# s-elkazdadi/ddp-pinocchio

Measured on AMD Instinct MI355X. Metric: DDP iterations/sec (fwd+bwd sweep), Talos nq=38 T=200, higher is better.
Workload: dtype f64

## Files before the change

### ddp_pinocchio_amd/csrc/lin_static.hip

```cpp
#include <float.h>
#include <math.h>
#include <stdlib.h>

#include <type_traits>
#include <utility>

#include "internal.h"
#include "lin_common.h"
#include "rbd.h"

#ifndef DEV_NO_EMIT
#define DEV_NO_EMIT 0
#endif
namespace {

struct TopoTalos38 {
  static constexpr int N = 38;
  static constexpr int parent[N] = {-1, 0, 1, 2, 3, 4,
                                    5, 6, 7, 8, 9, 10,
                                    5, 12, 13, 14, 15, 16,
                                    5, 18,
                                    19, 20, 21, 22, 23, 24, 25, 26,
                                    19, 28, 29, 30, 31, 32, 33, 34,
                                    19, 36};
  static constexpr int prismatic[N] = {1, 1, 1, 0, 0, 0, 0, 0, 0, 0, 0, 0, 0, 0, 0, 0, 0, 0, 0,
                                       0, 0, 0, 0, 0, 0, 0, 0, 0, 0, 0, 0, 0, 0, 0, 0, 0, 0, 0};
};

struct TopoChain6 {
  static constexpr int N = 6;
  static constexpr int parent[N] = {-1, 0, 1, 2, 3, 4};
  static constexpr int prismatic[N] = {0, 0, 0, 0, 0, 0};
};

}
#include "topo_extra.h"
namespace {

template <class T> constexpr bool has_child(int k) {
  for (int c = k + 1; c < T::N; ++c) if (T::parent[c] == k) return true;
  return false;
}
template <class T> constexpr int largest_child(int k) {
  int r = -1;
  for (int c = k + 1; c < T::N; ++c) if (T::parent[c] == k) r = c;
  return r;
}
template <class T> constexpr bool first_contrib(int k) { return T::parent[k] >= 0 && largest_child<T>(T::parent[k]) == k; }

template <class T>
bool topo_matches(const DevModel& m) {
  if (m.kind != DDP_HIP_MODEL_TREE || m.nv != T::N) return false;
  for (int i = 0; i < T::N; ++i)
    if (m.parent[i] != T::parent[i] || (m.jtype[i] == DDP_HIP_JOINT_PRISMATIC) != (T::prismatic[i] != 0)) return false;
  return true;
}

template <class T>
struct TauState {
  double acc[T::N][6];
  double uu[T::N];
};

template <class T, int K, int QS>
__device__ __forceinline__ void tau_up(const DevModel& m, const double* __restrict__ qc, const double* __restrict__ vc,
                                       double tauK, TauState<T>& s) {
  constexpr int o = T::prismatic[K] ? 3 : 0;
  const double* E = qc + K * QS;
  const double* r = E + 9;
  const double* U = E + 12;
  const double dinv = E[18];
  const double* pA0 = vc + K * rbd::VC_STRIDE + 6;
  const double* Iac = vc + K * rbd::VC_STRIDE + 12;
  const double* a = m.axis[K];
  double pAi[6];
  if constexpr (has_child<T>(K)) {
#pragma unroll
    for (int k = 0; k < 6; ++k) pAi[k] = s.acc[K][k];
  } else {
#pragma unroll
    for (int k = 0; k < 6; ++k) pAi[k] = pA0[k];
  }
  double sp = 0;
#pragma unroll
  for (int k = 0; k < 3; ++k) sp += a[k] * pAi[o + k];
  const double ui = tauK - sp;
  s.uu[K] = ui;
  constexpr int par = T::parent[K];
  if constexpr (par >= 0) {
    double pa[6], fp[6];
#pragma unroll
    for (int k = 0; k < 6; ++k) pa[k] = pAi[k] + Iac[k] + U[k] * (ui * dinv);
    rbd::xform_force_T(E, r, pa, fp);
    if constexpr (first_contrib<T>(K)) {
      const double* pp0 = vc + par * rbd::VC_STRIDE + 6;
#pragma unroll
      for (int k = 0; k < 6; ++k) s.acc[par][k] = pp0[k] + fp[k];
    } else {
#pragma unroll
      for (int k = 0; k < 6; ++k) s.acc[par][k] += fp[k];
    }
  }
  if constexpr (QS == rbd::QC_STRIDE || (K % 2) == 0) __builtin_amdgcn_sched_barrier(0);
}

template <class T, int K, int QS>
__device__ __forceinline__ void tau_down(const DevModel& m, const double* __restrict__ qc, const double* __restrict__ vc,
                                         TauState<T>& s) {
  constexpr int o = T::prismatic[K] ? 3 : 0;
  const double* E = qc + K * QS;
  const double* r = E + 9;
  const double* U = E + 12;
  const double dinv = E[18];
  const double* cb = vc + K * rbd::VC_STRIDE;
  double ap[6];
  constexpr int par = T::parent[K];
  if constexpr (par >= 0) rbd::xform_motion(E, r, s.acc[par], ap);
  else {
    const double a0[6] = {0, 0, 0, -m.gravity[0], -m.gravity[1], -m.gravity[2]};
    rbd::xform_motion(E, r, a0, ap);
  }
  double sum = 0;
#pragma unroll
  for (int k = 0; k < 6; ++k) { ap[k] += cb[k]; sum += U[k] * ap[k]; }
  const double qd = (s.uu[K] - sum) * dinv;
  s.uu[K] = qd;
  if constexpr (has_child<T>(K)) {
    const double* a = m.axis[K];
#pragma unroll
    for (int k = 0; k < 6; ++k) s.acc[K][k] = ap[k];
    s.acc[K][o] += a[0] * qd; s.acc[K][o + 1] += a[1] * qd; s.acc[K][o + 2] += a[2] * qd;
  }
  if constexpr (QS == rbd::QC_STRIDE || (K % 2) == 0) __builtin_amdgcn_sched_barrier(0);
}

template <class T, int QS, class TauFn, int... Ks>
__device__ __forceinline__ void tau_up_all(const DevModel& m, const double* __restrict__ qc, const double* __restrict__ vc, TauFn tau,
                                           TauState<T>& s, std::integer_sequence<int, Ks...>) {
  (tau_up<T, T::N - 1 - Ks, QS>(m, qc, vc, tau(T::N - 1 - Ks), s), ...);
}
template <class T, int QS, int HI, class TauFn, int... Ks>
__device__ __forceinline__ void tau_up_range(const DevModel& m, const double* __restrict__ qc, const double* __restrict__ vc, TauFn tau,
                                             TauState<T>& s, std::integer_sequence<int, Ks...>) {
  (tau_up<T, HI - Ks, QS>(m, qc, vc, tau(HI - Ks), s), ...);
}
template <class T, int QS, int... Ks>
__device__ __forceinline__ void tau_down_all(const DevModel& m, const double* __restrict__ qc, const double* __restrict__ vc,
                                             TauState<T>& s, std::integer_sequence<int, Ks...>) {
  (tau_down<T, Ks, QS>(m, qc, vc, s), ...);
}

constexpr int PS = 20;
template <int NV>
__device__ __forceinline__ void stage_placements(double* sp, const double* __restrict__ qc, int lane) {
  for (int idx = lane; idx < NV * 19; idx += LBS) {
    const int K = idx / 19, e = idx - K * 19;
    sp[K * PS + e] = qc[K * rbd::QC_STRIDE + e];
  }
}

template <int BYTES>
__device__ __forceinline__ unsigned int warm_block(const double* base, int lane) {
  typedef unsigned int u4 __attribute__((ext_vector_type(4)));
  const char* b = reinterpret_cast<const char*>(base);
  unsigned int sink = 0;
#pragma unroll
  for (int off = 0; off < BYTES; off += LBS * 16) {
    int o = off + lane * 16;
    o = o < BYTES - 16 ? o : BYTES - 16;
    const u4 v = *reinterpret_cast<const u4*>(b + o);
    sink ^= v.x ^ v.y ^ v.z ^ v.w;
  }
  return sink;
}

template <class T> constexpr bool parents_at_least(int from, int lo) {
  for (int k = from; k < T::N; ++k) if (T::parent[k] < lo) return false;
  return true;
}
template <class T> constexpr int stage_split() {
  for (int kh = T::N / 2; kh > 0; --kh) if (parents_at_least<T>(kh + 1, kh)) return kh;
  return 0;
}

template <int NV, int K0, int K1, bool WITH_V = true>
struct StageRegs {
  static constexpr int NPW = (K1 - K0) * 19, NVW = WITH_V ? (K1 - K0) * rbd::VC_STRIDE : 0;
  static constexpr int CP = (NPW + LBS - 1) / LBS, CV = (NVW + LBS - 1) / LBS;
  double rp[CP], rv[CV > 0 ? CV : 1];
  __device__ __forceinline__ void load(const double* __restrict__ qc, const double* __restrict__ vc, int lane) {
#pragma unroll
    for (int c = 0; c < CP; ++c) {
      int idx = c * LBS + lane;
      idx = idx < NPW ? idx : NPW - 1;
      const int K = K0 + idx / 19, e = idx % 19;
      rp[c] = qc[K * rbd::QC_STRIDE + e];
    }
#pragma unroll
    for (int c = 0; c < CV; ++c) {
      int idx = c * LBS + lane;
      idx = idx < NVW ? idx : NVW - 1;
      rv[c] = vc[K0 * rbd::VC_STRIDE + idx];
    }
  }
  __device__ __forceinline__ void park(double* sp, double* sv, int lane) const {
#pragma unroll
    for (int c = 0; c < CP; ++c) {
      int idx = c * LBS + lane;
      idx = idx < NPW ? idx : NPW - 1;
      const int K = K0 + idx / 19, e = idx % 19;
      sp[K * PS + e] = rp[c];
    }
#pragma unroll
    for (int c = 0; c < CV; ++c) {
      int idx = c * LBS + lane;
      idx = idx < NVW ? idx : NVW - 1;
      sv[K0 * rbd::VC_STRIDE + idx] = rv[c];
    }
  }
};

__device__ __forceinline__ void tri_index(int64_t q, int Wd, int& ii, int& jj) {
  int a = (int)floor(((2.0 * Wd - 1.0) - sqrt((2.0 * Wd - 1.0) * (2.0 * Wd - 1.0) - 8.0 * (double)q)) * 0.5);
  if (a < 0) a = 0;
  while ((int64_t)a * (2 * Wd - a - 1) / 2 > q) --a;
  while ((int64_t)(a + 1) * (2 * Wd - a - 2) / 2 <= q) ++a;
  ii = a;
  jj = (int)(q - (int64_t)a * (2 * Wd - a - 1) / 2) + a + 1;
}

template <int NV, int NP = LBS>
struct OutStage {
  double qdd[NP * (NV + 1)];
  int pij[NP];
};

template <int NV, int NP>
__device__ __forceinline__ void offdiag_emit(const LinParams& p, OutStage<NV, NP>& S, bool valid, int i, int j, int64_t bt,
                                             const double* __restrict__ xg, double dt, int pass = 0) {
  constexpr int n = 2 * NV, mm = NV;
  constexpr int RW = 16, NJ = (n + RW - 1) / RW, GRP = LBS / RW, PPG = NP / GRP, NB = NP == LBS ? 2 : 1;
  static_assert(PPG % NB == 0, "points per group");
  const double eps = sqrt(sqrt(DBL_EPSILON));
  const double eps2 = eps * eps;
  const int lane = threadIdx.x;
  if (lane / NP == pass) S.pij[lane % NP] = i | (j << 8) | ((valid ? 1 : 0) << 16);
  double* const fxx = p.fxx + bt * n * n * n;
  double* const fux = p.fux + bt * n * mm * n;
  double* const fuu = p.fuu + bt * n * mm * mm;
  const double* const fxb = p.fx + bt * n * n;
  const double* const fub = p.fu + bt * n * mm;
  __syncthreads();
  const int kk = lane % RW, grp = lane / RW;
  const double* f0 = p.f_val + bt * n;
  double f0k[NJ], xk[NJ], xvk[NJ];
#pragma unroll
  for (int jx = 0; jx < NJ; ++jx) {
    const int k = kk + RW * jx;
    const int kc = k < n ? k : n - 1;
    f0k[jx] = f0[kc];
    xk[jx] = xg[kc];
    xvk[jx] = kc < NV ? xg[NV + kc] : 0.0;
  }
  if (DEV_NO_EMIT) return;
  for (int pt = 0; pt < PPG; pt += NB) {
    double a1[NB][NJ], a2[NB][NJ], d1[NB][NJ], d2[NB][NJ];
    double* o0[NB];
    double* o1[NB];
    int ie[NB], je[NB], ee[NB];
#pragma unroll
    for (int u = 0; u < NB; ++u) {
      const int e = (pt + u) * GRP + grp;
      ee[u] = e;
      const int pk = S.pij[e];
      const int i1 = pk & 255, j1 = (pk >> 8) & 255;
      ie[u] = i1;
      je[u] = j1;
      const bool at_x_1 = i1 < n, at_x_2 = j1 < n;
      const int idx_1 = at_x_1 ? i1 : i1 - n, idx_2 = at_x_2 ? j1 : j1 - n;
      double* tensor;
      int L;
      if (at_x_1) { if (at_x_2) { tensor = fxx; L = n; } else { tensor = fux; L = mm; } }
      else { tensor = fuu; L = mm; }
      o0[u] = (pk >> 16) ? tensor + (int64_t)idx_2 * n + (int64_t)idx_1 * n * L : nullptr;
      o1[u] = ((pk >> 16) && at_x_1 == at_x_2 && !p.skip_qv_mirror) ? tensor + (int64_t)idx_1 * n + (int64_t)idx_2 * n * L : nullptr;
      if (o0[u]) {
        const double* q0 = at_x_1 ? fxb + (int64_t)idx_1 * n : fub + (int64_t)idx_1 * n;
        const double* q1 = at_x_2 ? fxb + (int64_t)idx_2 * n : fub + (int64_t)idx_2 * n;
        const double* q2 = at_x_1 ? fxx + (int64_t)idx_1 * n + (int64_t)idx_1 * n * n : fuu + (int64_t)idx_1 * n + (int64_t)idx_1 * n * mm;
        const double* q3 = at_x_2 ? fxx + (int64_t)idx_2 * n + (int64_t)idx_2 * n * n : fuu + (int64_t)idx_2 * n + (int64_t)idx_2 * n * mm;
#pragma unroll
        for (int jx = 0; jx < NJ; ++jx) {
          const int k = kk + RW * jx;
          const int kc = k < n ? k : n - 1;
          a1[u][jx] = q0[kc]; a2[u][jx] = q1[kc]; d1[u][jx] = q2[kc]; d2[u][jx] = q3[kc];
        }
      }
    }
#pragma unroll
    for (int u = 0; u < NB; ++u) {
      if (!o0[u]) continue;
#pragma unroll
      for (int jx = 0; jx < NJ; ++jx) {
        const int k = kk + RW * jx;
        if (k >= n) continue;
        if (p.skip_top && k < NV && !((ie[u] < n && ie[u] % NV == k) || (je[u] < n && je[u] % NV == k))) continue;
        double xs = k == ie[u] ? xk[jx] + eps : xk[jx];
        if (k == je[u]) xs = xs + eps;
        double fv;
        if (k < NV) {
          double xv = (NV + k) == ie[u] ? xvk[jx] + eps : xvk[jx];
          if (NV + k == je[u]) xv = xv + eps;
          const double vo = dt * xv;
          fv = xs + vo;
        } else {
          fv = xs + S.qdd[ee[u] * (NV + 1) + (k - NV)] * dt;
        }
        double df = fv - f0k[jx];
        df -= eps * a1[u][jx];
        df -= eps * a2[u][jx];
        df *= 2;
        const double val = 0.5 * (df / eps2 - d1[u][jx] - d2[u][jx]);
        o0[u][k] = val;
        if (o1[u]) o1[u][k] = val;
      }
    }
  }
}

template <int NV>
struct RowStage {
  double q[(NV + 2) * (NV + 1)];
};

template <int NV, bool DIAG_ROW, class ST>
__device__ __forceinline__ void rowblock_emit(const ST& S, int lane, int i, int jb, double* __restrict__ out, double* __restrict__ mirror,
                                              int64_t mstride, const double* __restrict__ a2, const double* __restrict__ d2, int64_t dstride,
                                              double dt, const double* __restrict__ f0g, const double* __restrict__ a1g,
                                              double* __restrict__ d1g, const double* __restrict__ xg, bool skip_top = false) {
  constexpr int n = 2 * NV, RW = 16, NJ = (n + RW - 1) / RW, CG = LBS / RW, NIT = (NV + CG - 1) / CG;
  const int r1 = i % NV;
  const double eps = sqrt(sqrt(DBL_EPSILON));
  const double eps2 = eps * eps;
  const int kk = lane % RW, cg = lane / RW;
  double xk[NJ], xvk[NJ], f0k[NJ], a1k[NJ], d1k[NJ];
#pragma unroll
  for (int j = 0; j < NJ; ++j) {
    const int k = kk + RW * j;
    const int kc = k < n ? k : n - 1;
    f0k[j] = f0g[kc];
    a1k[j] = a1g[kc];
    double x = xg[kc];
    if (kc == i) x = x + eps;
    xk[j] = x;
    double xv = xg[kc < NV ? NV + kc : kc];
    if (NV + kc == i) xv = xv + eps;
    xvk[j] = xv;
    if constexpr (DIAG_ROW) {
      double fv;
      if (kc < NV) {
        const double vo = dt * xv;
        fv = x + vo;
      } else {
        fv = x + S.q[NV * (NV + 1) + (kc - NV)] * dt;
      }
      double df = fv - f0k[j];
      df -= eps * a1k[j];
      df *= 2;
      const double dd = df / eps2;
      d1k[j] = dd;
      if (cg == 0 && k < n && !(skip_top && k < NV && k != r1)) d1g[k] = dd;
    } else {
      d1k[j] = d1g[kc];
    }
  }
  double va2[2][NJ], vd2[2][NJ];
  auto fetch = [&](int it, double (&A)[NJ], double (&D)[NJ]) {
    const int c = it * CG + cg;
    const int cc = c < NV ? c : NV - 1;
#pragma unroll
    for (int j = 0; j < NJ; ++j) {
      const int k = kk + RW * j;
      const int kc = k < n ? k : n - 1;
      A[j] = a2[kc + cc * n];
      D[j] = d2[kc + cc * dstride];
    }
  };
  auto form = [&](int it, const double (&A)[NJ], const double (&D)[NJ]) {
    const int c = it * CG + cg;
    const bool cv = c < NV;
    const int cc = cv ? c : NV - 1;
    const int jp = jb + cc;
#pragma unroll
    for (int j = 0; j < NJ; ++j) {
      const int k = kk + RW * j;
      if (!(cv && k < n)) continue;
      if (skip_top && k < NV && k != r1 && !(jp < n && jp % NV == k)) continue;
      double x = xk[j];
      if (k == jp) x = x + eps;
      double fv;
      if (k < NV) {
        double xv = xvk[j];
        if (NV + k == jp) xv = xv + eps;
        const double vo = dt * xv;
        fv = x + vo;
      } else {
        fv = x + S.q[cc * (NV + 1) + (k - NV)] * dt;
      }
      double df = fv - f0k[j];
      df -= eps * a1k[j];
      df -= eps * A[j];
      df *= 2;
      const double val = 0.5 * (df / eps2 - d1k[j] - D[j]);
      out[k + c * n] = val;
      if (mirror) mirror[k + c * mstride] = val;
    }
  };
  if (DEV_NO_EMIT) return;
  fetch(0, va2[0], vd2[0]);
  for (int it = 0; it < NIT; it += 2) {
    if (it + 1 < NIT) fetch(it + 1, va2[1], vd2[1]);
    form(it, va2[0], vd2[0]);
    if (it + 1 < NIT) {
      if (it + 2 < NIT) fetch(it + 2, va2[0], vd2[0]);
      form(it + 1, va2[1], vd2[1]);
    }
  }
}

template <class T, bool ROWS>
__global__ __launch_bounds__(LBS, ROWS ? 1 : 3) void lin_static_tau_kernel(LinParams p) {
  constexpr int nv = T::N, n = 2 * nv;
  constexpr int TRI = nv * (nv - 1) / 2, GU = (TRI + LBS - 1) / LBS, G = ROWS ? 2 * nv : GU;
  const int64_t bt = blockIdx.x / G;
  const int g = (int)(blockIdx.x % G) + (ROWS ? 0 : 2 * nv);
  const int lane = threadIdx.x;
  const int64_t Tn = p.d.T;
  const int b = (int)(bt / Tn);
  const int64_t t = bt % Tn;
  const DevModel& m = *p.model;
  int i, j, cfg, vcfg;
  bool valid;
  if (g < nv) { i = g; j = n + lane; cfg = 1 + g; vcfg = nv + 1 + g; valid = lane < nv; }
  else if (g < 2 * nv) { i = g; j = n + lane; cfg = 0; vcfg = 1 + (g - nv); valid = lane < nv; }
  else {
    const int pid = (g - 2 * nv) * LBS + lane;
    valid = pid < TRI;
    tri_index(valid ? pid : 0, nv, i, j);
    i += n; j += n; cfg = 0; vcfg = 0;
  }
  double eps = sqrt(sqrt(DBL_EPSILON));
  const double* __restrict__ qc = p.qcache + (bt * (nv + 1) + cfg) * (int64_t)nv * rbd::QC_STRIDE;
  const double* __restrict__ vc = p.vcache + (bt * (2 * nv + 1) + vcfg) * (int64_t)nv * rbd::VC_STRIDE;
  const double* __restrict__ xg = p.x + ((int64_t)b * (Tn + 1) + t) * n;
  const double* __restrict__ ug = p.u + ((int64_t)b * Tn + t) * nv;
  const int iu = i - n, ju = j - n;
  __shared__ union TauLds { double P[ROWS ? nv * PS + nv * rbd::VC_STRIDE : 1]; RowStage<nv> S; } s_lds;
  double* s_P = s_lds.P;
  unsigned int w = 0;
  double* s_V = s_P + nv * PS;
  constexpr int KH = ROWS ? stage_split<T>() : 0;
  StageRegs<nv, 0, (ROWS && KH > 0) ? KH : 1> lower;
  if constexpr (ROWS) {
    StageRegs<nv, KH, nv> upper;
    upper.load(qc, vc, lane);
    lower.load(qc, vc, lane);
    upper.park(s_P, s_V, lane);
    rbd::coop_sync<true>();
  } else {
    w = warm_block<nv * rbd::VC_STRIDE * 8>(vc, lane);
    w ^= warm_block<nv * rbd::QC_STRIDE * 8>(qc, lane);
  }
  if (w == 0x7fc01234u) eps = 0.0;
  TauState<T> s;
  auto tau = [&](int k) { double v = ug[k]; if (k == iu) v = v + eps; if (k == ju) v = v + eps; return v; };
  if constexpr (ROWS) {
    static_assert(!ROWS || parents_at_least<T>(KH + 1, KH), "the first half of the pass must not reach below record KH");
    tau_up_range<T, PS, nv - 1>(m, s_P, s_V, tau, s, std::make_integer_sequence<int, nv - 1 - KH>{});
    lower.park(s_P, s_V, lane);
    rbd::coop_sync<true>();
    tau_up_range<T, PS, KH>(m, s_P, s_V, tau, s, std::make_integer_sequence<int, KH + 1>{});
    tau_down_all<T, PS>(m, s_P, s_V, s, std::make_integer_sequence<int, nv>{});
  } else {
    tau_up_all<T, rbd::QC_STRIDE>(m, qc, vc, tau, s, std::make_integer_sequence<int, nv>{});
    tau_down_all<T, rbd::QC_STRIDE>(m, qc, vc, s, std::make_integer_sequence<int, nv>{});
  }
  __builtin_amdgcn_sched_barrier(0);
  typedef __attribute__((address_space(4))) const LinParams* kernarg_t;
  const kernarg_t kp = (kernarg_t)__builtin_amdgcn_kernarg_segment_ptr();
  if constexpr (ROWS) {
    RowStage<nv>& S = s_lds.S;
    const int mm = nv;
    __syncthreads();
    const int row = lane <= nv ? lane : nv + 1;
#pragma unroll
    for (int k = 0; k < nv; ++k) S.q[row * (nv + 1) + k] = s.uu[k];
    __syncthreads();
    rowblock_emit<nv, true>(S, lane, i, n, kp->fux + bt * n * mm * n + (int64_t)i * n * mm, nullptr, 0, kp->fu + bt * n * mm,
                            kp->fuu + bt * n * mm * mm, (int64_t)n + (int64_t)n * mm, m.dt, kp->f_val + bt * n,
                            kp->fx + bt * n * n + (int64_t)i * n, kp->fxx + bt * n * n * n + (int64_t)i * n + (int64_t)i * n * n, xg, kp->skip_top != 0);
  } else {
    __shared__ OutStage<nv, LBS / 2> S;
    LinParams po;
    po.f_val = kp->f_val; po.fx = kp->fx; po.fu = kp->fu; po.fxx = kp->fxx; po.fux = kp->fux; po.fuu = kp->fuu; po.skip_qv_mirror = kp->skip_qv_mirror; po.skip_top = kp->skip_top;
    const double dt = m.dt;
#pragma unroll 1
    for (int pass = 0; pass < 2; ++pass) {
      if (pass) __syncthreads();
      if (lane / (LBS / 2) == pass) {
#pragma unroll
        for (int k = 0; k < nv; ++k) S.qdd[(lane % (LBS / 2)) * (nv + 1) + k] = s.uu[k];
      }
      offdiag_emit<nv, LBS / 2>(po, S, valid, i, j, bt, xg, dt, pass);
    }
  }
}

template <class T> constexpr int n_children(int k) {
  int c = 0;
  for (int j = k + 1; j < T::N; ++j) if (T::parent[j] == k) ++c;
  return c;
}
template <class T> constexpr bool chain_start(int k) { return T::parent[k] < 0 || T::parent[k] != k - 1 || n_children<T>(T::parent[k]) > 1; }
template <class T> constexpr bool chain_end(int k) { return k == T::N - 1 || chain_start<T>(k + 1); }
template <class T> constexpr int chain_first(int k) { while (!chain_start<T>(k)) --k; return k; }
template <class T> constexpr int max_chain() {
  int best = 1;
  for (int k = 0; k < T::N; ++k)
    if (chain_end<T>(k)) { const int len = k - chain_first<T>(k) + 1; if (len > best) best = len; }
  return best;
}

template <class T>
struct VelState {
  double vel[T::N][6];
  double acc[T::N][6];
  double uu[T::N];
};

template <int UQS_, int QS_ = rbd::QC_STRIDE>
struct VelCtx {
  static constexpr int UQS = UQS_;
  static constexpr int QS = QS_;
  const DevModel* m;
  const double* qp;
  const double* __restrict__ qc;
  const double* __restrict__ xg;
  const double* __restrict__ ug;
  double* uq;
  int i, j;
  double eps;
  template <int K> __device__ __forceinline__ const double* er(double*) const { return qp + K * QS; }
  template <int K> __device__ __forceinline__ const double* er_down(double* b) const { return er<K>(b); }
  template <int K> __device__ __forceinline__ const double* ud() const { return qp + K * QS + 12; }
  template <int K> __device__ __forceinline__ void ia_cb(const double*, const double* cb, double* Iac) const { rbd::sym6_mv(qc + K * rbd::QC_STRIDE + 19, cb, Iac); }
  template <int K> __device__ __forceinline__ const double* ud_down() const { return ud<K>(); }
};

template <int NV, class C>
__device__ __forceinline__ double lane_v(const C& c, int K) {
  double v = c.xg[NV + K];
  if (NV + K == c.i) v = v + c.eps;
  if (NV + K == c.j) v = v + c.eps;
  return v;
}

template <class T, int K, class C>
__device__ __forceinline__ void joint_vel(const C& c, const double* vel_par, double* vel) {
  constexpr int o = T::prismatic[K] ? 3 : 0;
  double Pb[12];
  const double* E = c.template er<K>(Pb);
  const double* r = E + 9;
  const double* a = c.m->axis[K];
  const double vK = lane_v<T::N>(c, K);
  double vJ[6] = {0, 0, 0, 0, 0, 0};
  vJ[o] = a[0] * vK; vJ[o + 1] = a[1] * vK; vJ[o + 2] = a[2] * vK;
  if constexpr (T::parent[K] >= 0) rbd::xform_motion(E, r, vel_par, vel);
  else {
#pragma unroll
    for (int k = 0; k < 6; ++k) vel[k] = 0.0;
  }
#pragma unroll
  for (int k = 0; k < 6; ++k) vel[k] += vJ[k];
}
template <class T, int K, class C>
__device__ __forceinline__ void vel_from_root(const C& c, double* vel) {
  if constexpr (T::parent[K] >= 0) {
    double vp[6];
    vel_from_root<T, T::parent[K]>(c, vp);
    joint_vel<T, K>(c, vp, vel);
  } else {
    joint_vel<T, K>(c, nullptr, vel);
  }
}
template <class T, int K, class C>
__device__ __forceinline__ void bias_force0(const C& c, const double* vel, double* pA) {
  double Iv[6];
  rbd::sym6_mv(c.m->I6[K], vel, Iv);
  rbd::crf(vel, Iv, pA);
}

template <class T, int K, int E, class C>
__device__ __forceinline__ void chain_down(const C& c, VelState<T>& s) {
  if constexpr (T::parent[K] >= 0) joint_vel<T, K>(c, s.vel[T::parent[K]], s.vel[K]);
  else joint_vel<T, K>(c, nullptr, s.vel[K]);
  __builtin_amdgcn_sched_barrier(0);
  if constexpr (K < E) chain_down<T, K + 1, E>(c, s);
}

template <class T, int K, int F, class C>
__device__ __forceinline__ void chain_up(const C& c, VelState<T>& s) {
  constexpr int o = T::prismatic[K] ? 3 : 0;
  double Pb[12];
  const double* E = c.template er<K>(Pb);
  const double* r = E + 9;
  const double* U = c.template ud<K>();
  const double dinv = U[6];
  const double* a = c.m->axis[K];
  double pAi[6];
  if constexpr (has_child<T>(K)) {
#pragma unroll
    for (int k = 0; k < 6; ++k) pAi[k] = s.acc[K][k];
  } else {
    bias_force0<T, K>(c, s.vel[K], pAi);
  }
  double sp = 0;
#pragma unroll
  for (int k = 0; k < 3; ++k) sp += a[k] * pAi[o + k];
  const double ui = c.ug[K] - sp;
  if constexpr (C::UQS == 0) s.uu[K] = ui; else c.uq[K * C::UQS] = ui;
  constexpr int par = T::parent[K];
  if constexpr (par >= 0) {
    const double vK = lane_v<T::N>(c, K);
    double vJ[6] = {0, 0, 0, 0, 0, 0}, cb[6], pa[6], Iac[6], fp[6];
    vJ[o] = a[0] * vK; vJ[o + 1] = a[1] * vK; vJ[o + 2] = a[2] * vK;
    rbd::crm(s.vel[K], vJ, cb);
    c.template ia_cb<K>(U, cb, Iac);
#pragma unroll
    for (int k = 0; k < 6; ++k) pa[k] = pAi[k] + Iac[k] + U[k] * (ui * dinv);
    rbd::xform_force_T(E, r, pa, fp);
    if constexpr (first_contrib<T>(K)) {
      double p0[6];
      bias_force0<T, par>(c, s.vel[par], p0);
#pragma unroll
      for (int k = 0; k < 6; ++k) s.acc[par][k] = p0[k] + fp[k];
    } else {
#pragma unroll
      for (int k = 0; k < 6; ++k) s.acc[par][k] += fp[k];
    }
  }
  __builtin_amdgcn_sched_barrier(0);
  if constexpr (K > F) chain_up<T, K - 1, F>(c, s);
}

template <class T, int K, class C>
__device__ __forceinline__ void chain_at(const C& c, VelState<T>& s) {
  if constexpr (chain_end<T>(K)) {
    constexpr int F = chain_first<T>(K), P = T::parent[F];
    if constexpr (P >= 0) {
      if constexpr (first_contrib<T>(F) && n_children<T>(P) > 1) vel_from_root<T, P>(c, s.vel[P]);
    }
    chain_down<T, F, K>(c, s);
    chain_up<T, K, F>(c, s);
  }
}
template <class T, class C, int... Ks>
__device__ __forceinline__ void vel_up_all(const C& c, VelState<T>& s, std::integer_sequence<int, Ks...>) {
  (chain_at<T, T::N - 1 - Ks>(c, s), ...);
}

template <class T, int K, class C>
__device__ __forceinline__ void vel_down(const C& c, VelState<T>& s) {
  constexpr int o = T::prismatic[K] ? 3 : 0;
  constexpr int par = T::parent[K];
  double Pb[12];
  const double* E = c.template er_down<K>(Pb);
  const double* r = E + 9;
  const double* U = c.template ud_down<K>();
  const double dinv = U[6];
  const double* a = c.m->axis[K];
  const double vK = lane_v<T::N>(c, K);
  double vJ[6] = {0, 0, 0, 0, 0, 0}, vel[6], cb[6], ap[6];
  vJ[o] = a[0] * vK; vJ[o + 1] = a[1] * vK; vJ[o + 2] = a[2] * vK;
  if constexpr (par >= 0) {
    rbd::xform_motion(E, r, s.vel[par], vel);
    rbd::xform_motion(E, r, s.acc[par], ap);
  } else {
    const double a0[6] = {0, 0, 0, -c.m->gravity[0], -c.m->gravity[1], -c.m->gravity[2]};
#pragma unroll
    for (int k = 0; k < 6; ++k) vel[k] = 0.0;
    rbd::xform_motion(E, r, a0, ap);
  }
#pragma unroll
  for (int k = 0; k < 6; ++k) vel[k] += vJ[k];
  rbd::crm(vel, vJ, cb);
  double sum = 0;
#pragma unroll
  for (int k = 0; k < 6; ++k) { ap[k] += cb[k]; sum += U[k] * ap[k]; }
  double ui;
  if constexpr (C::UQS == 0) ui = s.uu[K]; else ui = c.uq[K * C::UQS];
  const double qd = (ui - sum) * dinv;
  if constexpr (C::UQS == 0) s.uu[K] = qd; else c.uq[K * C::UQS] = qd;
  if constexpr (has_child<T>(K)) {
#pragma unroll
    for (int k = 0; k < 6; ++k) { s.vel[K][k] = vel[k]; s.acc[K][k] = ap[k]; }
    s.acc[K][o] += a[0] * qd; s.acc[K][o + 1] += a[1] * qd; s.acc[K][o + 2] += a[2] * qd;
  }
  __builtin_amdgcn_sched_barrier(0);
}
template <class T, class C, int... Ks>
__device__ __forceinline__ void vel_down_all(const C& c, VelState<T>& s, std::integer_sequence<int, Ks...>) {
  (vel_down<T, Ks>(c, s), ...);
}

template <class T, bool ROWS>
__global__ __launch_bounds__(LBS, ROWS ? 3 : 1) void lin_static_vel_kernel(LinParams p) {
  constexpr int nv = T::N, n = 2 * nv;
  constexpr int TRI = nv * (nv - 1) / 2, GU = (TRI + LBS - 1) / LBS, G = ROWS ? nv : GU;
  const int64_t bt = blockIdx.x / G;
  const int g = (int)(blockIdx.x % G);
  const int lane = threadIdx.x;
  const int64_t Tn = p.d.T;
  const int b = (int)(bt / Tn);
  const int64_t t = bt % Tn;
  int i, j, cfg;
  bool valid;
  if (ROWS) { i = g; j = nv + lane; cfg = 1 + g; valid = lane < nv; }
  else {
    const int pid = g * LBS + lane;
    valid = pid < TRI;
    tri_index(valid ? pid : 0, nv, i, j);
    i += nv; j += nv; cfg = 0;
  }
  using Stage = typename std::conditional<ROWS, RowStage<nv>, OutStage<nv>>::type;
  __shared__ union VelLds { Stage S; double P[ROWS ? nv * rbd::QC_STRIDE : 1]; } s_lds;
  Stage& S = s_lds.S;
  double* s_P = s_lds.P;
  VelCtx<ROWS ? 0 : 1, rbd::QC_STRIDE> c;
  c.m = p.model;
  c.qc = p.qcache + (bt * (nv + 1) + cfg) * (int64_t)nv * rbd::QC_STRIDE;
  c.qp = ROWS ? s_P : c.qc;
  c.xg = p.x + ((int64_t)b * (Tn + 1) + t) * n;
  c.ug = p.u + ((int64_t)b * Tn + t) * nv;
  c.i = i; c.j = j;
  c.eps = sqrt(sqrt(DBL_EPSILON));
  if constexpr (ROWS) c.uq = nullptr;
  else c.uq = &S.qdd[lane * (nv + 1)];
  if constexpr (ROWS) {
    constexpr int NW = nv * rbd::QC_STRIDE, CW = (NW + LBS - 1) / LBS;
    double rq[CW];
#pragma unroll
    for (int r = 0; r < CW; ++r) { const int idx = r * LBS + lane; rq[r] = c.qc[idx < NW ? idx : NW - 1]; }
#pragma unroll
    for (int r = 0; r < CW; ++r) { const int idx = r * LBS + lane; s_P[idx < NW ? idx : NW - 1] = rq[r]; }
    c.qc = s_P;
    rbd::coop_sync<true>();
  } else {
    const unsigned int w = warm_block<nv * rbd::QC_STRIDE * 8>(c.qc, lane);
    if (w == 0x7fc01234u) c.eps = 0.0;
  }
  VelState<T> s;
  vel_up_all<T>(c, s, std::make_integer_sequence<int, nv>{});
  vel_down_all<T>(c, s, std::make_integer_sequence<int, nv>{});
  __builtin_amdgcn_sched_barrier(0);
  typedef __attribute__((address_space(4))) const LinParams* kernarg_t;
  const kernarg_t kp = (kernarg_t)__builtin_amdgcn_kernarg_segment_ptr();
  const double dt = c.m->dt;
  if constexpr (ROWS) {
    double* fxx = kp->fxx + bt * n * n * n;
    const double* fxb = kp->fx + bt * n * n;
    __syncthreads();
    const int row = valid ? lane : nv;
#pragma unroll
    for (int k = 0; k < nv; ++k) S.q[row * (nv + 1) + k] = s.uu[k];
    __syncthreads();
    rowblock_emit<nv, false>(S, lane, i, nv, fxx + (int64_t)nv * n + (int64_t)i * n * n,
                             kp->skip_qv_mirror ? nullptr : fxx + (int64_t)i * n + (int64_t)nv * n * n, (int64_t)n * n,
                             fxb + (int64_t)nv * n, fxx + (int64_t)nv * n + (int64_t)nv * n * n, (int64_t)n + (int64_t)n * n, dt,
                             kp->f_val + bt * n, fxb + (int64_t)i * n, fxx + (int64_t)i * n + (int64_t)i * n * n, c.xg, kp->skip_top != 0);
  } else {
    LinParams po;
    po.f_val = kp->f_val; po.fx = kp->fx; po.fu = kp->fu; po.fxx = kp->fxx; po.fux = kp->fux; po.fuu = kp->fuu; po.skip_qv_mirror = kp->skip_qv_mirror; po.skip_top = kp->skip_top;
    offdiag_emit<nv, LBS>(po, S, valid, i, j, bt, c.xg, dt);
  }
}

constexpr int WS_PER_JOINT = 8;

template <class T>
struct CfgState {
  double vel[T::N][6];
  double accP[T::N][6];
  double accI[T::N][21];
  double w[2][WS_PER_JOINT];
};

struct CfgCtx {
  const DevModel* __restrict__ m;
  const double* __restrict__ qc0;
  const double* __restrict__ xg;
  const double* __restrict__ ug;
  double* __restrict__ W;
  double* lvel;
  int i, j;
  const double* own;
};

template <int K, int NV>
__device__ __forceinline__ void lane_placement(const CfgCtx& c, double* P) {
  const double* base = c.qc0 + K * rbd::QC_STRIDE;
  const double* pert = c.own ? c.own : c.qc0 + ((int64_t)(1 + K) * NV + K) * rbd::QC_STRIDE;
  const bool own = K == c.i || K == c.j;
#pragma unroll
  for (int e = 0; e < 12; ++e) P[e] = own ? pert[e] : base[e];
}

template <class T, int K>
__device__ __forceinline__ void cfg_joint_vel(const CfgCtx& c, const double* P, const double* vel_par, double* vel) {
  constexpr int o = T::prismatic[K] ? 3 : 0;
  const double* a = c.m->axis[K];
  const double vK = c.xg[T::N + K];
  double vJ[6] = {0, 0, 0, 0, 0, 0};
  vJ[o] = a[0] * vK; vJ[o + 1] = a[1] * vK; vJ[o + 2] = a[2] * vK;
  if constexpr (T::parent[K] >= 0) rbd::xform_motion(P, P + 9, vel_par, vel);
  else {
#pragma unroll
    for (int k = 0; k < 6; ++k) vel[k] = 0.0;
  }
#pragma unroll
  for (int k = 0; k < 6; ++k) vel[k] += vJ[k];
}
template <class T, int K>
__device__ __forceinline__ void cfg_vel_from_root(const CfgCtx& c, double* vel) {
  double P[12];
  lane_placement<K, T::N>(c, P);
  if constexpr (T::parent[K] >= 0) {
    double vp[6];
    cfg_vel_from_root<T, T::parent[K]>(c, vp);
    cfg_joint_vel<T, K>(c, P, vp, vel);
  } else {
    cfg_joint_vel<T, K>(c, P, nullptr, vel);
  }
}
template <int K>
__device__ __forceinline__ void cfg_bias_force0(const CfgCtx& c, const double* vel, double* pA) {
  double Iv[6];
  rbd::sym6_mv(c.m->I6[K], vel, Iv);
  rbd::crf(vel, Iv, pA);
}

template <class T, int K, int F, int E>
__device__ __forceinline__ void cfg_chain_down(const CfgCtx& c, CfgState<T>& s, double* cur) {
  double P[12], vel[6];
  lane_placement<K, T::N>(c, P);
  if constexpr (T::parent[K] >= 0) cfg_joint_vel<T, K>(c, P, cur, vel);
  else cfg_joint_vel<T, K>(c, P, nullptr, vel);
#pragma unroll
  for (int k = 0; k < 6; ++k) { cur[k] = vel[k]; c.lvel[((K - F) * 6 + k) * LBS] = vel[k]; }
  __builtin_amdgcn_sched_barrier(0);
  if constexpr (K < E) cfg_chain_down<T, K + 1, F, E>(c, s, cur);
}
template <class T, int K, int F>
__device__ __forceinline__ void chain_vel_load(const CfgCtx& c, const CfgState<T>& s, double* vel) {
  if constexpr (K >= F) {
#pragma unroll
    for (int k = 0; k < 6; ++k) vel[k] = c.lvel[((K - F) * 6 + k) * LBS];
  } else {
#pragma unroll
    for (int k = 0; k < 6; ++k) vel[k] = s.vel[K][k];
  }
}

template <class T, int K, int F>
__device__ __forceinline__ void cfg_chain_up(const CfgCtx& c, CfgState<T>& s) {
  constexpr int o = T::prismatic[K] ? 3 : 0;
  const double* a = c.m->axis[K];
  double IA[21], pAi[6], U[6], velK[6];
  chain_vel_load<T, K, F>(c, s, velK);
  if constexpr (has_child<T>(K)) {
#pragma unroll
    for (int k = 0; k < 21; ++k) IA[k] = s.accI[K][k];
#pragma unroll
    for (int k = 0; k < 6; ++k) pAi[k] = s.accP[K][k];
  } else {
#pragma unroll
    for (int k = 0; k < 21; ++k) IA[k] = c.m->I6[K][k];
    cfg_bias_force0<K>(c, velK, pAi);
  }
  double d = 0, sp = 0;
#pragma unroll
  for (int r = 0; r < 6; ++r) U[r] = IA[rbd::sidx(r, o)] * a[0] + IA[rbd::sidx(r, o + 1)] * a[1] + IA[rbd::sidx(r, o + 2)] * a[2];
#pragma unroll
  for (int k = 0; k < 3; ++k) { d += a[k] * U[o + k]; sp += a[k] * pAi[o + k]; }
  const double dinv = 1.0 / d;
  const double ui = c.ug[K] - sp;
#pragma unroll
  for (int k = 0; k < 6; ++k) c.W[(K * WS_PER_JOINT + k) * LBS] = U[k];
  c.W[(K * WS_PER_JOINT + 6) * LBS] = dinv;
  c.W[(K * WS_PER_JOINT + 7) * LBS] = ui;
  constexpr int par = T::parent[K];
  if constexpr (par >= 0) {
    double P[12], Ia[21], vJ[6] = {0, 0, 0, 0, 0, 0}, cb[6], pa[6], Iac[6], fp[6];
    lane_placement<K, T::N>(c, P);
    const double vK = c.xg[T::N + K];
    vJ[o] = a[0] * vK; vJ[o + 1] = a[1] * vK; vJ[o + 2] = a[2] * vK;
#pragma unroll
    for (int r = 0; r < 6; ++r)
#pragma unroll
      for (int cc = 0; cc <= r; ++cc) Ia[rbd::sidx(r, cc)] = IA[rbd::sidx(r, cc)] - U[r] * U[cc] * dinv;
    rbd::crm(velK, vJ, cb);
    rbd::sym6_mv(Ia, cb, Iac);
#pragma unroll
    for (int k = 0; k < 6; ++k) pa[k] = pAi[k] + Iac[k] + U[k] * (ui * dinv);
    if constexpr (first_contrib<T>(K)) {
      double velP[6];
      chain_vel_load<T, par, F>(c, s, velP);
#pragma unroll
      for (int k = 0; k < 21; ++k) s.accI[par][k] = c.m->I6[par][k];
      cfg_bias_force0<par>(c, velP, s.accP[par]);
    }
    rbd::add_xtix(P, P + 9, Ia, s.accI[par]);
    rbd::xform_force_T(P, P + 9, pa, fp);
#pragma unroll
    for (int k = 0; k < 6; ++k) s.accP[par][k] += fp[k];
  }
  __builtin_amdgcn_sched_barrier(0);
  if constexpr (K > F) cfg_chain_up<T, K - 1, F>(c, s);
}

template <class T, int K>
__device__ __forceinline__ void cfg_chain_at(const CfgCtx& c, CfgState<T>& s) {
  if constexpr (chain_end<T>(K)) {
    constexpr int F = chain_first<T>(K), P = T::parent[F];
    if constexpr (P >= 0) {
      if constexpr (first_contrib<T>(F) && n_children<T>(P) > 1) cfg_vel_from_root<T, P>(c, s.vel[P]);
    }
    double cur[6] = {0, 0, 0, 0, 0, 0};
    if constexpr (P >= 0) {
#pragma unroll
      for (int k = 0; k < 6; ++k) cur[k] = s.vel[P][k];
    }
    cfg_chain_down<T, F, F, K>(c, s, cur);
    cfg_chain_up<T, K, F>(c, s);
  }
}
template <class T, int... Ks>
__device__ __forceinline__ void cfg_up_all(const CfgCtx& c, CfgState<T>& s, std::integer_sequence<int, Ks...>) {
  (cfg_chain_at<T, T::N - 1 - Ks>(c, s), ...);
}

template <int STRIDE_>
struct CfgDownOut { double* uq; static constexpr int STRIDE = STRIDE_; };

template <class T, int K, class O>
__device__ __forceinline__ void cfg_down(const CfgCtx& c, CfgState<T>& s, const O& out) {
  constexpr int o = T::prismatic[K] ? 3 : 0;
  constexpr int par = T::parent[K];
  if constexpr (K + 1 < T::N) {
#pragma unroll
    for (int e = 0; e < WS_PER_JOINT; ++e) s.w[(K + 1) & 1][e] = c.W[((K + 1) * WS_PER_JOINT + e) * LBS];
  }
  const double* U = s.w[K & 1];
  const double dinv = s.w[K & 1][6], ui = s.w[K & 1][7];
  const double* a = c.m->axis[K];
  const double vK = c.xg[T::N + K];
  double P[12], vJ[6] = {0, 0, 0, 0, 0, 0}, vel[6], cb[6], ap[6];
  lane_placement<K, T::N>(c, P);
  vJ[o] = a[0] * vK; vJ[o + 1] = a[1] * vK; vJ[o + 2] = a[2] * vK;
  if constexpr (par >= 0) {
    rbd::xform_motion(P, P + 9, s.vel[par], vel);
    rbd::xform_motion(P, P + 9, s.accP[par], ap);
  } else {
    const double a0[6] = {0, 0, 0, -c.m->gravity[0], -c.m->gravity[1], -c.m->gravity[2]};
#pragma unroll
    for (int k = 0; k < 6; ++k) vel[k] = 0.0;
    rbd::xform_motion(P, P + 9, a0, ap);
  }
#pragma unroll
  for (int k = 0; k < 6; ++k) vel[k] += vJ[k];
  rbd::crm(vel, vJ, cb);
  double sum = 0;
#pragma unroll
  for (int k = 0; k < 6; ++k) { ap[k] += cb[k]; sum += U[k] * ap[k]; }
  const double qd = (ui - sum) * dinv;
  out.uq[K * (O::STRIDE == LBS ? LBS : 1)] = qd;
  if constexpr (has_child<T>(K)) {
#pragma unroll
    for (int k = 0; k < 6; ++k) { s.vel[K][k] = vel[k]; s.accP[K][k] = ap[k]; }
    s.accP[K][o] += a[0] * qd; s.accP[K][o + 1] += a[1] * qd; s.accP[K][o + 2] += a[2] * qd;
  }
  __builtin_amdgcn_sched_barrier(0);
}
template <class T, class O, int... Ks>
__device__ __forceinline__ void cfg_down_all(const CfgCtx& c, CfgState<T>& s, const O& out, std::integer_sequence<int, Ks...>) {
  (cfg_down<T, Ks>(c, s, out), ...);
}

template <class T>
__device__ __forceinline__ void cfg_setup(CfgCtx& c, const LinParams& p, const DevModel* __restrict__ model, const double* __restrict__ qcache,
                                          const double* __restrict__ xs, const double* __restrict__ us, double* __restrict__ ws,
                                          int64_t bt0, int64_t& bt, bool& valid) {
  constexpr int nv = T::N, n = 2 * nv;
  constexpr int TRI = nv * (nv - 1) / 2, GU = (TRI + LBS - 1) / LBS;
  bt = bt0 + blockIdx.x / GU;
  const int g = (int)(blockIdx.x % GU);
  const int lane = threadIdx.x;
  const int64_t Tn = p.d.T;
  const int b = (int)(bt / Tn);
  const int64_t t = bt % Tn;
  const int pid = g * LBS + lane;
  valid = pid < TRI;
  tri_index(valid ? pid : 0, nv, c.i, c.j);
  c.m = model;
  c.qc0 = qcache + (bt * (nv + 1)) * (int64_t)nv * rbd::QC_STRIDE;
  c.xg = xs + ((int64_t)b * (Tn + 1) + t) * n;
  c.ug = us + ((int64_t)b * Tn + t) * nv;
  c.W = ws + (int64_t)blockIdx.x * (nv * WS_PER_JOINT * LBS) + lane;
  c.own = nullptr;
}

template <class T>
__global__ __launch_bounds__(LBS) void lin_static_cfg_up_kernel(LinParams p, const DevModel* __restrict__ model, const double* __restrict__ qcache,
                                                                const double* __restrict__ xs, const double* __restrict__ us,
                                                                double* __restrict__ ws, int64_t bt0) {
  constexpr int nv = T::N;
  constexpr int MAXCH = max_chain<T>();
  __shared__ double s_vel[MAXCH * 6 * LBS];
  CfgCtx c;
  int64_t bt;
  bool valid;
  cfg_setup<T>(c, p, model, qcache, xs, us, ws, bt0, bt, valid);
  c.lvel = s_vel + threadIdx.x;
  CfgState<T> s;
  cfg_up_all<T>(c, s, std::make_integer_sequence<int, nv>{});
}

template <class T>
__global__ __launch_bounds__(LBS) void lin_static_cfg_down_kernel(LinParams p, const DevModel* __restrict__ model, const double* __restrict__ qcache,
                                                                  const double* __restrict__ xs, const double* __restrict__ us,
                                                                  double* __restrict__ ws, int64_t bt0) {
  constexpr int nv = T::N;
  __shared__ OutStage<nv> S;
  CfgCtx c;
  int64_t bt;
  bool valid;
  cfg_setup<T>(c, p, model, qcache, xs, us, ws, bt0, bt, valid);
  c.lvel = nullptr;
  CfgState<T> s;
#pragma unroll
  for (int e = 0; e < WS_PER_JOINT; ++e) s.w[0][e] = c.W[e * LBS];
  CfgDownOut<nv + 1> o{&S.qdd[threadIdx.x * (nv + 1)]};
  cfg_down_all<T>(c, s, o, std::make_integer_sequence<int, nv>{});
  __builtin_amdgcn_sched_barrier(0);
  typedef __attribute__((address_space(4))) const LinParams* kernarg_t;
  const kernarg_t kp = (kernarg_t)__builtin_amdgcn_kernarg_segment_ptr();
  LinParams po;
  po.f_val = kp->f_val; po.fx = kp->fx; po.fu = kp->fu; po.fxx = kp->fxx; po.fux = kp->fux; po.fuu = kp->fuu; po.skip_qv_mirror = kp->skip_qv_mirror; po.skip_top = kp->skip_top;
  offdiag_emit<nv, LBS>(po, S, valid, c.i, c.j, bt, c.xg, model->dt);
}

constexpr int SREC = 13;

template <class T>
struct SpineTab {
  static constexpr int N = T::N, TRI = N * (N - 1) / 2;
  static_assert(N >= 2 && N <= 64, "ancestor masks are 64 bits wide");
  unsigned long long mask[N];
  unsigned long long anc[N];
  int depth[N];
  int nrec;
  short pi[TRI], pj[TRI];
  short top[TRI];
  int rbase[TRI], rstride[TRI];
};
template <class T>
constexpr SpineTab<T> make_spine_tab() {
  SpineTab<T> t{};
  for (int k = 0; k < T::N; ++k)
    for (int a = T::parent[k]; a >= 0; a = T::parent[a]) { ++t.depth[k]; t.mask[a] |= 1ull << k; t.anc[k] |= 1ull << a; }
  int cnt[T::N + 2] = {}, start[T::N + 2] = {}, goff[T::N + 2] = {};
  for (int i = 0; i < T::N; ++i)
    for (int j = i + 1; j < T::N; ++j) {
      int a = T::parent[i];
      while (a >= 0 && !((t.mask[a] >> j) & 1)) a = T::parent[a];
      ++cnt[a + 1];
    }
// ... 655 lines not shown
```

Measured before the change: 683.1.

## Stage placement caches in LDS for off-diagonal tau and vel kernels

The off-diagonal (non-ROWS) tau and velocity kernels now copy the per-block q/v placement caches into shared memory through a register-staged load and barrier, as the row kernels already do. This replaces the prior warm-block cache-prefetch trick that read from global memory. The output staging now shares an LDS union with the placement buffer and emits in two half-block passes, which shrinks LDS use. The vel kernel's launch bounds are raised to allow 3 blocks per CU. This adds extra barriers and LDS traffic and risks register pressure under the tighter launch bound.

```diff
diff --git a/ddp_pinocchio_amd/csrc/lin_static.hip b/ddp_pinocchio_amd/csrc/lin_static.hip
--- a/ddp_pinocchio_amd/csrc/lin_static.hip
+++ b/ddp_pinocchio_amd/csrc/lin_static.hip
@@ -157,21 +157,6 @@
     const int K = idx / 19, e = idx - K * 19;
     sp[K * PS + e] = qc[K * rbd::QC_STRIDE + e];
   }
-}
-
-template <int BYTES>
-__device__ __forceinline__ unsigned int warm_block(const double* base, int lane) {
-  typedef unsigned int u4 __attribute__((ext_vector_type(4)));
-  const char* b = reinterpret_cast<const char*>(base);
-  unsigned int sink = 0;
-#pragma unroll
-  for (int off = 0; off < BYTES; off += LBS * 16) {
-    int o = off + lane * 16;
-    o = o < BYTES - 16 ? o : BYTES - 16;
-    const u4 v = *reinterpret_cast<const u4*>(b + o);
-    sink ^= v.x ^ v.y ^ v.z ^ v.w;
-  }
-  return sink;
 }
 
 template <class T> constexpr bool parents_at_least(int from, int lo) {
@@ -449,47 +434,45 @@
     tri_index(valid ? pid : 0, nv, i, j);
     i += n; j += n; cfg = 0; vcfg = 0;
   }
-  double eps = sqrt(sqrt(DBL_EPSILON));
+  const double eps = sqrt(sqrt(DBL_EPSILON));
   const double* __restrict__ qc = p.qcache + (bt * (nv + 1) + cfg) * (int64_t)nv * rbd::QC_STRIDE;
   const double* __restrict__ vc = p.vcache + (bt * (2 * nv + 1) + vcfg) * (int64_t)nv * rbd::VC_STRIDE;
   const double* __restrict__ xg = p.x + ((int64_t)b * (Tn + 1) + t) * n;
   const double* __restrict__ ug = p.u + ((int64_t)b * Tn + t) * nv;
   const int iu = i - n, ju = j - n;
-  __shared__ union TauLds { double P[ROWS ? nv * PS + nv * rbd::VC_STRIDE : 1]; RowStage<nv> S; } s_lds;
+  using Stage = typename std::conditional<ROWS, RowStage<nv>, OutStage<nv, LBS / 2>>::type;
+  __shared__ union TauLds { double P[nv * PS + nv * rbd::VC_STRIDE]; Stage S; } s_lds;
   double* s_P = s_lds.P;
-  unsigned int w = 0;
   double* s_V = s_P + nv * PS;
-  constexpr int KH = ROWS ? stage_split<T>() : 0;
-  StageRegs<nv, 0, (ROWS && KH > 0) ? KH : 1> lower;
+  TauState<T> s;
+  auto tau = [&](int k) { double v = ug[k]; if (k == iu) v = v + eps; if (k == ju) v = v + eps; return v; };
   if constexpr (ROWS) {
+    constexpr int KH = stage_split<T>();
     StageRegs<nv, KH, nv> upper;
+    StageRegs<nv, 0, (KH > 0) ? KH : 1> lower;
     upper.load(qc, vc, lane);
     lower.load(qc, vc, lane);
     upper.park(s_P, s_V, lane);
     rbd::coop_sync<true>();
-  } else {
-    w = warm_block<nv * rbd::VC_STRIDE * 8>(vc, lane);
-    w ^= warm_block<nv * rbd::QC_STRIDE * 8>(qc, lane);
-  }
-  if (w == 0x7fc01234u) eps = 0.0;
-  TauState<T> s;
-  auto tau = [&](int k) { double v = ug[k]; if (k == iu) v = v + eps; if (k == ju) v = v + eps; return v; };
-  if constexpr (ROWS) {
-    static_assert(!ROWS || parents_at_least<T>(KH + 1, KH), "the first half of the pass must not reach below record KH");
+    static_assert(parents_at_least<T>(KH + 1, KH), "the first half of the pass must not reach below record KH");
     tau_up_range<T, PS, nv - 1>(m, s_P, s_V, tau, s, std::make_integer_sequence<int, nv - 1 - KH>{});
     lower.park(s_P, s_V, lane);
     rbd::coop_sync<true>();
     tau_up_range<T, PS, KH>(m, s_P, s_V, tau, s, std::make_integer_sequence<int, KH + 1>{});
     tau_down_all<T, PS>(m, s_P, s_V, s, std::make_integer_sequence<int, nv>{});
   } else {
-    tau_up_all<T, rbd::QC_STRIDE>(m, qc, vc, tau, s, std::make_integer_sequence<int, nv>{});
-    tau_down_all<T, rbd::QC_STRIDE>(m, qc, vc, s, std::make_integer_sequence<int, nv>{});
+    StageRegs<nv, 0, nv> all;
+    all.load(qc, vc, lane);
+    all.park(s_P, s_V, lane);
+    rbd::coop_sync<true>();
+    tau_up_all<T, PS>(m, s_P, s_V, tau, s, std::make_integer_sequence<int, nv>{});
+    tau_down_all<T, PS>(m, s_P, s_V, s, std::make_integer_sequence<int, nv>{});
   }
   __builtin_amdgcn_sched_barrier(0);
   typedef __attribute__((address_space(4))) const LinParams* kernarg_t;
   const kernarg_t kp = (kernarg_t)__builtin_amdgcn_kernarg_segment_ptr();
   if constexpr (ROWS) {
-    RowStage<nv>& S = s_lds.S;
+    Stage& S = s_lds.S;
     const int mm = nv;
     __syncthreads();
     const int row = lane <= nv ? lane : nv + 1;
@@ -500,10 +483,11 @@
                             kp->fuu + bt * n * mm * mm, (int64_t)n + (int64_t)n * mm, m.dt, kp->f_val + bt * n,
                             kp->fx + bt * n * n + (int64_t)i * n, kp->fxx + bt * n * n * n + (int64_t)i * n + (int64_t)i * n * n, xg, kp->skip_top != 0);
   } else {
-    __shared__ OutStage<nv, LBS / 2> S;
+    Stage& S = s_lds.S;
     LinParams po;
     po.f_val = kp->f_val; po.fx = kp->fx; po.fu = kp->fu; po.fxx = kp->fxx; po.fux = kp->fux; po.fuu = kp->fuu; po.skip_qv_mirror = kp->skip_qv_mirror; po.skip_top = kp->skip_top;
     const double dt = m.dt;
+    __syncthreads();
 #pragma unroll 1
     for (int pass = 0; pass < 2; ++pass) {
       if (pass) __syncthreads();
@@ -714,7 +698,7 @@
 }
 
 template <class T, bool ROWS>
-__global__ __launch_bounds__(LBS, ROWS ? 3 : 1) void lin_static_vel_kernel(LinParams p) {
+__global__ __launch_bounds__(LBS, 3) void lin_static_vel_kernel(LinParams p) {
   constexpr int nv = T::N, n = 2 * nv;
   constexpr int TRI = nv * (nv - 1) / 2, GU = (TRI + LBS - 1) / LBS, G = ROWS ? nv : GU;
   const int64_t bt = blockIdx.x / G;
@@ -732,21 +716,20 @@
     tri_index(valid ? pid : 0, nv, i, j);
     i += nv; j += nv; cfg = 0;
   }
-  using Stage = typename std::conditional<ROWS, RowStage<nv>, OutStage<nv>>::type;
-  __shared__ union VelLds { Stage S; double P[ROWS ? nv * rbd::QC_STRIDE : 1]; } s_lds;
+  using Stage = typename std::conditional<ROWS, RowStage<nv>, OutStage<nv, LBS / 2>>::type;
+  __shared__ union VelLds { Stage S; double P[nv * rbd::QC_STRIDE]; } s_lds;
   Stage& S = s_lds.S;
   double* s_P = s_lds.P;
-  VelCtx<ROWS ? 0 : 1, rbd::QC_STRIDE> c;
+  VelCtx<0, rbd::QC_STRIDE> c;
   c.m = p.model;
   c.qc = p.qcache + (bt * (nv + 1) + cfg) * (int64_t)nv * rbd::QC_STRIDE;
-  c.qp = ROWS ? s_P : c.qc;
+  c.qp = s_P;
   c.xg = p.x + ((int64_t)b * (Tn + 1) + t) * n;
   c.ug = p.u + ((int64_t)b * Tn + t) * nv;
   c.i = i; c.j = j;
   c.eps = sqrt(sqrt(DBL_EPSILON));
-  if constexpr (ROWS) c.uq = nullptr;
-  else c.uq = &S.qdd[lane * (nv + 1)];
-  if constexpr (ROWS) {
+  c.uq = nullptr;
+  {
     constexpr int NW = nv * rbd::QC_STRIDE, CW = (NW + LBS - 1) / LBS;
     double rq[CW];
 #pragma unroll
@@ -755,9 +738,6 @@
     for (int r = 0; r < CW; ++r) { const int idx = r * LBS + lane; s_P[idx < NW ? idx : NW - 1] = rq[r]; }
     c.qc = s_P;
     rbd::coop_sync<true>();
-  } else {
-    const unsigned int w = warm_block<nv * rbd::QC_STRIDE * 8>(c.qc, lane);
-    if (w == 0x7fc01234u) c.eps = 0.0;
   }
   VelState<T> s;
   vel_up_all<T>(c, s, std::make_integer_sequence<int, nv>{});
@@ -781,7 +761,16 @@
   } else {
     LinParams po;
     po.f_val = kp->f_val; po.fx = kp->fx; po.fu = kp->fu; po.fxx = kp->fxx; po.fux = kp->fux; po.fuu = kp->fuu; po.skip_qv_mirror = kp->skip_qv_mirror; po.skip_top = kp->skip_top;
-    offdiag_emit<nv, LBS>(po, S, valid, i, j, bt, c.xg, dt);
+    __syncthreads();
+#pragma unroll 1
+    for (int pass = 0; pass < 2; ++pass) {
+      if (pass) __syncthreads();
+      if (lane / (LBS / 2) == pass) {
+#pragma unroll
+        for (int k = 0; k < nv; ++k) S.qdd[(lane % (LBS / 2)) * (nv + 1) + k] = s.uu[k];
+      }
+      offdiag_emit<nv, LBS / 2>(po, S, valid, i, j, bt, c.xg, dt, pass);
+    }
   }
 }
 
```

Result: faster. 711.6, median of 6 (+4.2%).
